# alpc91/SGRL

Measured on AMD Instinct MI355X. Metric: env-steps/sec (whole node) + SET-actor fwd us/step, 3d_walker mix @8192 envs/GPU, higher is better.
Workload: dtype f64 (dynamics) / f32 (SET actor, obs); 1 GPU; 3D_Walker++ 8 variants x 1024 envs per GPU (config 3), random U(-1,1) actions, auto-reset, SET actor forward on every step, random-init weights; envs_per_gpu=8192, obs_max_len=287, action_max_len=21, replay_gather=none (single rank)

## Files before the change

### sgrl_amd/_lib.py

```python
import ctypes
import os
import subprocess

_HERE = os.path.dirname(os.path.abspath(__file__))
LIB_PATH = os.environ.get("SGRL_HIP_LIB", os.path.join(_HERE, "libsgrl_hip.so"))
CSRC = os.path.join(_HERE, "csrc")
SOURCES = ["engine.hip", "set_actor.hip", "train_gemm.hip", "render.hip", "swat_actor.hip", "smp_actor.hip", "replay_sample.hip", "eval_record.hip", "explore_actions.hip", "scene.hip", "mlp_actor.hip", "mlp_train.hip", "mlp_optim.hip", "mlp_batch.hip", "smp_train.hip", "td3_loss.hip", "dropout.hip"]

_lib = None

_i32p = ctypes.POINTER(ctypes.c_int32)
_f64p = ctypes.POINTER(ctypes.c_double)


class SgrlError(RuntimeError):
    pass


HDR_DIM_FIELDS = (1, 2, 3, 4, 5, 6, 7, 8, 9, 16, 18)
LIGHT_NV = 12
ITAB_GLOBAL = set(x for x in os.environ.get("SGRL_BUILD_ITAB_GLOBAL", "humanoid").split(",") if x and x != "none")
PAIR_NV = {"walker": 15, "hopper": 15}


def default_max_rows(model):
    return 256


def spec_families():
    from . import mjcf, model_pack
    from .env_spec import env_spec_for
    fam = {}
    for n in mjcf.list_assets():
        m = mjcf.load_asset(n)
        ib, _ = model_pack.pack_model(m, spec=env_spec_for(n), max_rows=default_max_rows(m))
        d = tuple(int(ib[i]) for i in HDR_DIM_FIELDS)
        fam.setdefault(n.split("_")[1], set()).add(d)
    out = []
    for key in sorted(fam):
        itab = 1 if key in ITAB_GLOBAL else 0
        out.append((len(out), 2, [d + (0 if itab else (1 if d[3] <= PAIR_NV.get(key, LIGHT_NV) else 0),) for d in sorted(fam[key])], itab))
    for key in sorted(fam):
        light = sorted(d for d in fam[key] if d[3] <= LIGHT_NV)
        if light:
            out.append((len(out), 4, [d + (0,) for d in light], 0))
    return out


def hash_text(t):
    import zlib
    return zlib.crc32(t.encode())


def _write_if_changed(path, text):
    if not os.path.exists(path) or open(path).read() != text:
        with open(path, "w") as f:
            f.write(text)


def build(verbose=False):
    from concurrent.futures import ThreadPoolExecutor
    fams = spec_families()
    table = ("// generated by sgrl_amd/_lib.py build() from sgrl_amd/assets/models\n"
             "// SGRL_FAMILY(id, waves per SIMD, members, int tables in global memory)   SGRL_MEMBER(family, slot, nbody, njnt, nq, nv, nu, ngeom, npair, integrator, frame_skip, max_rows, solver, pair)\n")
    for i, w, dims, itab in fams:
        table += "SGRL_FAMILY(%d, %d, %d, %d)\n" % (i, w, len(dims), itab)
        table += "".join("SGRL_MEMBER(%d, %d, %s)\n" % (i, k, ", ".join(str(x) for x in d)) for k, d in enumerate(dims))
    _write_if_changed(os.path.join(CSRC, "spec_table.inc"), table)
    hdrs = [os.path.join(CSRC, f) for f in os.listdir(CSRC) if f.endswith((".h", ".inc"))]
    hdrs += [os.path.join(_HERE, "..", "include", f) for f in ("sgrl.h", "sgrl_model.h", "sgrl_set.h", "sgrl_swat.h", "sgrl_smp.h", "sgrl_train.h", "sgrl_render.h", "sgrl_replay.h", "sgrl_eval.h", "sgrl_explore.h", "sgrl_mlp.h")
             if os.path.exists(os.path.join(_HERE, "..", "include", f))]
    newest_hdr = max(os.path.getmtime(d) for d in hdrs)
    objdir = os.path.join(_HERE, "..", "build", "obj")
    os.makedirs(objdir, exist_ok=True)
    base = ["hipcc", "--offload-arch=gfx950", "-O3", "-std=c++17", "-fPIC", "-fno-slp-vectorize"]
    jobs = []
    for sname in SOURCES:
        src = os.path.join(CSRC, sname)
        if os.path.exists(src):
            jobs.append((os.path.join(objdir, sname.replace(".hip", ".o")), src, []))
    spec_src = os.path.join(CSRC, "step_spec.hip")
    for i, w, dims, itab in fams:
        members = ",".join("DimsFixed<%s>" % ",".join(str(x) for x in d) for d in dims)
        flags = ["-DSGRL_SPEC_ID=%d" % i, "-DSGRL_SPEC_WAVES=%d" % w, "-DSGRL_SPEC_FAMILY=" + members]
        if itab:
            flags.append("-DSGRL_ITAB_GLOBAL=1")
        tag = "%08x" % (hash_text(members + str(w) + ("g" if itab else "")) & 0xFFFFFFFF)
        jobs.append((os.path.join(objdir, "family_%d_%s.o" % (i, tag)), spec_src, flags))

    def compile_one(job):
        obj, src, flags = job
        if os.path.exists(obj) and os.path.getmtime(obj) >= max(newest_hdr, os.path.getmtime(src)):
            return False
        cmd = base + flags + ["-c", "-o", obj, src]
        if verbose:
            print(" ".join(cmd), flush=True)
        subprocess.check_call(cmd)
        return True

    with ThreadPoolExecutor(max_workers=min(8, os.cpu_count() or 1)) as pool:
        rebuilt = list(pool.map(compile_one, jobs))
    objs = [j[0] for j in jobs]
    for f in os.listdir(objdir):
        if f.endswith(".o") and os.path.join(objdir, f) not in objs:
            os.remove(os.path.join(objdir, f))
    if any(rebuilt) or not os.path.exists(LIB_PATH) or os.path.getmtime(LIB_PATH) < max(os.path.getmtime(o) for o in objs):
        cmd = ["hipcc", "--offload-arch=gfx950", "-shared", "-fPIC", "-o", LIB_PATH] + objs
        if verbose:
            print(" ".join(cmd[:8]), "... (%d objects)" % len(objs), flush=True)
        subprocess.check_call(cmd)
    return LIB_PATH


def lib():
    global _lib
    if _lib is not None:
        return _lib
    if not os.path.exists(LIB_PATH):
        raise SgrlError("HIP extension %s is missing: run `python -c 'import __graft_entry__ as g; g.build()'` "
                        "(no CPU fallback exists)" % LIB_PATH)
    import torch
    try:
        L = ctypes.CDLL(LIB_PATH)
    except OSError as e:
        raise SgrlError("cannot load %s: %s" % (LIB_PATH, e))
    L.sgrl_last_error.restype = ctypes.c_char_p
    L.sgrl_version.restype = ctypes.c_char_p
    L.sgrl_engine_create.restype = ctypes.c_int
    L.sgrl_engine_create.argtypes = [ctypes.c_int, ctypes.POINTER(_i32p), _i32p, ctypes.POINTER(_f64p), _i32p, _i32p,
                                     ctypes.c_int, ctypes.c_int, ctypes.c_uint64, ctypes.c_uint32, ctypes.c_int,
                                     ctypes.POINTER(ctypes.c_void_p)]
    L.sgrl_engine_destroy.argtypes = [ctypes.c_void_p]
    L.sgrl_engine_destroy.restype = None
    for name in ("sgrl_num_envs", "sgrl_record_stride", "sgrl_lds_bytes", "sgrl_launch_groups", "sgrl_fixed_dim_groups", "sgrl_paired_envs"):
        getattr(L, name).argtypes = [ctypes.c_void_p]
        getattr(L, name).restype = ctypes.c_int
    vp = ctypes.c_void_p
    L.sgrl_reset.argtypes = [vp, vp, vp, vp]
    L.sgrl_step.argtypes = [vp, vp, vp, vp, vp, vp, vp, vp, vp, ctypes.c_int, vp]
    L.sgrl_refresh.argtypes = [vp, vp, vp, vp]
    L.sgrl_get_records.argtypes = [vp, vp, vp]
    L.sgrl_set_records.argtypes = [vp, vp, vp]
    L.sgrl_time_steps.argtypes = [vp, vp, vp, vp, vp, ctypes.c_int, vp, ctypes.POINTER(ctypes.c_float)]
    ci = ctypes.c_int
    L.sgrl_pack_transitions.argtypes = [vp, ci, vp, ci, vp, ci, vp, vp, vp, vp, vp, vp, ci, ci, ci, vp]
    L.sgrl_ingest_rows.argtypes = [vp, ci, ci, ci, vp, vp, ci, vp]
    L.sgrl_ingest_block.argtypes = [vp, ci, ci, ci, vp, ci, vp, vp, vp, vp, vp]
    L.sgrl_round_record.argtypes = [vp, vp, vp, vp, vp, vp, vp, vp, vp, ci, ci, vp]
    L.sgrl_ingest_ws_words.argtypes = [ci]
    L.sgrl_ingest_ws_words.restype = ctypes.c_int64
    _lib = L
    return L


EXPLORE_GAUSS, EXPLORE_UNIFORM = 0, 1


def bind_explore(L):
    if getattr(L, "_explore_bound", False):
        return L
    vp, ci, cf = ctypes.c_void_p, ctypes.c_int, ctypes.c_float
    L.sgrl_explore_actions.argtypes = [vp, ci, vp, ci, vp, ci, ci, ctypes.c_int64, ctypes.c_uint64, ctypes.c_uint64, ci, cf, cf, cf, vp]
    L.sgrl_explore_actions.restype = ci
    L.sgrl_explore_actions_launches.argtypes = []
    L.sgrl_explore_actions_launches.restype = ci
    L.sgrl_explore_last_error.argtypes = []
    L.sgrl_explore_last_error.restype = ctypes.c_char_p
    L._explore_bound = True
    return L


EXPORTS = ["sgrl_engine_create", "sgrl_engine_destroy", "sgrl_num_envs", "sgrl_record_stride", "sgrl_lds_bytes", "sgrl_launch_groups", "sgrl_fixed_dim_groups", "sgrl_paired_envs",
           "sgrl_reset", "sgrl_step", "sgrl_get_records", "sgrl_set_records", "sgrl_refresh", "sgrl_time_steps", "sgrl_pack_transitions", "sgrl_round_record", "sgrl_ingest_rows", "sgrl_ingest_block", "sgrl_ingest_ws_words",
           "sgrl_last_error", "sgrl_version"]


def check(rc, what):
    if rc != 0:
        raise SgrlError("%s failed (%d): %s" % (what, rc, lib().sgrl_last_error().decode()))
```

### sgrl_amd/csrc/wave_hip.h

```cpp
#pragma once
#include <hip/hip_runtime.h>

#include "../../include/sgrl_model.h"

namespace sgrl {

template <int CTRL>
__device__ __forceinline__ double dpp_move(double x) {
  int lo = __double2loint(x), hi = __double2hiint(x);
  lo = __builtin_amdgcn_update_dpp(0, lo, CTRL, 0xF, 0xF, false);
  hi = __builtin_amdgcn_update_dpp(0, hi, CTRL, 0xF, 0xF, false);
  return __hiloint2double(hi, lo);
}
__device__ __forceinline__ double read_lane(double x, int l) {
  const int lo = __builtin_amdgcn_readlane(__double2loint(x), l);
  const int hi = __builtin_amdgcn_readlane(__double2hiint(x), l);
  return __hiloint2double(hi, lo);
}
__device__ __forceinline__ double wave_sum(double x) {
  x += dpp_move<0xB1>(x);
  x += dpp_move<0x4E>(x);
  x += dpp_move<0x141>(x);
  x += dpp_move<0x140>(x);
  return (read_lane(x, 0) + read_lane(x, 16)) + (read_lane(x, 32) + read_lane(x, 48));
}
__device__ __forceinline__ double wave_max(double x) {
  x = fmax(x, dpp_move<0xB1>(x));
  x = fmax(x, dpp_move<0x4E>(x));
  x = fmax(x, dpp_move<0x141>(x));
  x = fmax(x, dpp_move<0x140>(x));
  return fmax(fmax(read_lane(x, 0), read_lane(x, 16)), fmax(read_lane(x, 32), read_lane(x, 48)));
}

struct DimsAny {
  static constexpr bool kFixed = false;
  static constexpr bool kPair = false;
  __device__ static __forceinline__ void apply(int32_t*) {}
  template <class M> __device__ static __forceinline__ int hdr_const(const M& m, int idx) { return m.hdr[idx]; }
};
struct DimsAny;
template <int NB, int NJ, int NQ, int NV, int NU, int NG, int NP, int INTEG, int FSKIP, int MAXROWS, int SOLVER, int PAIR = 0>
struct DimsFixed {
  static constexpr bool kFixed = true;
  static constexpr int kNv = NV;
  static constexpr bool kPair = PAIR != 0;
  static_assert(PAIR == 0 || NV <= 15, "two-environments-per-wavefront instances are built for at most 15 dofs");
  __device__ static __forceinline__ void apply(int32_t* hdr) {
    hdr[SGRL_H_NBODY] = NB; hdr[SGRL_H_NJNT] = NJ; hdr[SGRL_H_NQ] = NQ; hdr[SGRL_H_NV] = NV; hdr[SGRL_H_NU] = NU;
    hdr[SGRL_H_NGEOM] = NG; hdr[SGRL_H_NPAIR] = NP; hdr[SGRL_H_INTEGRATOR] = INTEG; hdr[SGRL_H_FRAME_SKIP] = FSKIP;
    hdr[SGRL_H_MAX_ROWS] = MAXROWS; hdr[SGRL_H_SOLVER] = SOLVER;
  }
  template <class M> __device__ static __forceinline__ int hdr_const(const M& m, int idx) {
    return idx == SGRL_H_INTEGRATOR ? INTEG : (idx == SGRL_H_SOLVER ? SOLVER : (idx == SGRL_H_FRAME_SKIP ? FSKIP : m.hdr[idx]));
  }
};

typedef double sgrl_v4d __attribute__((ext_vector_type(4)));
#ifndef SGRL_AFF_MFMA_MIN
#define SGRL_AFF_MFMA_MIN 8
#endif
#ifndef SGRL_TRMM_MFMA_MIN
#define SGRL_TRMM_MFMA_MIN 9
#endif

template <int NVCAP, class D = DimsAny>
struct HipWaveT {
  static constexpr bool kFixedDims = D::kFixed;
  template <class M> __device__ static __forceinline__ int hdr_const(const M& m, int idx) { return D::hdr_const(m, idx); }
  int lane;
#ifdef SGRL_PHASE_PROF
  long long t_last = 0;
  unsigned long long* prof = nullptr;
  __device__ __forceinline__ void tick(int id) {
    const long long t = __builtin_readcyclecounter();
    if (id >= 0 && prof && lane == 0) prof[id] += (unsigned long long)(t - t_last);
    t_last = __builtin_readcyclecounter();
  }
#endif
  __device__ __forceinline__ HipWaveT() : lane(threadIdx.x & 63) {}
  __device__ __forceinline__ void fence_lane() { asm volatile("" : "+v"(lane)); }
  template <class T> __device__ __forceinline__ T fenced(T v) {
    int t = __builtin_amdgcn_readfirstlane((int)(unsigned)(__UINTPTR_TYPE__)v);
    asm volatile("" : "+s"(t));
    return (T)(__UINTPTR_TYPE__)(unsigned)t;
  }
  template <class F> __device__ __forceinline__ void lanes(int n, F f) {
    for (int i = lane; i < n; i += 64) f(i);
    __syncthreads();
  }
  template <class F> __device__ __forceinline__ void lanes_from(int lo, int hi, F f) {
    for (int i = lo + lane; i < hi; i += 64) f(i);
    __syncthreads();
  }
  template <class F> __device__ __forceinline__ double sum(int n, F f) {
    double p = 0.0;
    for (int i = lane; i < n; i += 64) p += f(i);
    return wave_sum(p);
  }
  __device__ __forceinline__ int pgs(int n_in, int nv_in, const double* Y, int ldy, const double* b, const double* R,
                                      const double* idg, double* f, double* v, int iters_in,
                                      double thresh) {
    const int n = __builtin_amdgcn_readfirstlane(n_in), nv = __builtin_amdgcn_readfirstlane(nv_in);
    const int iters = __builtin_amdgcn_readfirstlane(iters_in);
    const bool rowl = lane < n, dofl = lane < nv;
    double rb = rowl ? b[lane] : 0.0, rR = rowl ? R[lane] : 0.0;
    double ridg = rowl ? idg[lane] : 0.0, rf = rowl ? f[lane] : 0.0;
    const double rdg = rowl ? 1.0 / ridg : 0.0;
    double vv = 0.0;
    for (int r = 0; r < n; r++) {
      const double fr = read_lane(rf, r);
      if (dofl) vv += Y[r * ldy + lane] * fr;
    }
    int it = 0;
    for (; it < iters; it++) {
      double change = 0.0;
      double ynext = dofl ? Y[lane] : 0.0;
      for (int r = 0; r < n; r++) {
        const double y = ynext;
        if (r + 1 < n) ynext = dofl ? Y[(r + 1) * ldy + lane] : 0.0;
        const double dot = wave_sum(y * vv);
        const double fr = read_lane(rf, r);
        const double res = read_lane(rb, r) + read_lane(rR, r) * fr + dot;
        double fn = fr - res * read_lane(ridg, r);
        fn = fn < 0.0 ? 0.0 : fn;
        const double df = fn - fr;
        vv += y * df;
        if (lane == r) rf = fn;
        change = fmax(change, fabs(df) * read_lane(rdg, r));
      }
      if (change < thresh) { it++; break; }
    }
    if (rowl) f[lane] = rf;
    if (dofl) v[lane] = vv;
    __syncthreads();
    return it;
  }
  __device__ __forceinline__ int pgs_big(int n_in, int nv_in, const double* Y, int ldy, const double* b, const double* R,
                                          const double* idg, double* f, double* v, int iters_in, double thresh) {
    const int n = __builtin_amdgcn_readfirstlane(n_in), nv = __builtin_amdgcn_readfirstlane(nv_in);
    const int iters = __builtin_amdgcn_readfirstlane(iters_in);
    const bool dofl = lane < nv;
    const int dl = dofl ? lane : 0;
    double vv = 0.0;
    for (int r = 0; r < n; r++) {
      const double fr = f[r];
      const double y = Y[r * ldy + dl];
      if (dofl) vv += y * fr;
    }
    int it = 0;
    for (; it < iters; it++) {
      double change = 0.0;
      double yn = Y[dl], bn = b[0], Rn = R[0], in_ = idg[0], fn_ = f[0];
      for (int r = 0; r < n; r++) {
        const double y = dofl ? yn : 0.0, br = bn, Rr = Rn, ir = in_, fr = fn_;
        if (r + 1 < n) { yn = Y[(r + 1) * ldy + dl]; bn = b[r + 1]; Rn = R[r + 1]; in_ = idg[r + 1]; fn_ = f[r + 1]; }
        const double dot = wave_sum(y * vv);
        const double res = br + Rr * fr + dot;
        double fnew = fr - res * ir;
        fnew = fnew < 0.0 ? 0.0 : fnew;
        const double df = fnew - fr;
        vv += y * df;
        if (lane == 0) f[r] = fnew;
        change = fmax(change, fabs(df) / ir);
      }
      __syncthreads();
      if (change < thresh) { it++; break; }
    }
    if (dofl) v[lane] = vv;
    __syncthreads();
    return it;
  }
  template <int NMAX>
  __device__ __forceinline__ void chol_inv_reg(int n, double* P, double minval) {
    const bool act = lane < n;
    const int li = act ? lane : 0;
    double* rowp = P + li * (li + 1) / 2;
    double a[NMAX + 1];
#pragma unroll
    for (int k = 0; k < NMAX; k++) a[k + 1] = rowp[k < li ? k : li];
    double mydj = 0.0;
#pragma unroll
    for (int j = 0; j < NMAX; j++) {
      if (j < n) {
        const double c = a[j + 1];
        double pj = read_lane(c, j);
        pj = pj < minval ? minval : pj;
        const double dj = rsqrt(pj);
        const double l = c * dj;
        mydj = lane == j ? dj : mydj;
        const double lm = lane > j ? l * dj : 0.0;
        a[j] = lane == j ? 1.0 : 0.0;
#pragma unroll
        for (int c2 = 0; c2 <= j; c2++) a[c2] -= lm * read_lane(a[c2], j);
#pragma unroll
        for (int k = j + 1; k < NMAX; k++) a[k + 1] -= l * read_lane(l, k);
      }
    }
    if (act) {
#pragma unroll
      for (int k = NMAX - 1; k >= 0; k--) rowp[k < li ? k : li] = a[k] * mydj;
    }
    __syncthreads();
  }
  __device__ __forceinline__ bool chol_inv_packed(int n_in, double* P, double minval) {
    const int n = __builtin_amdgcn_readfirstlane(n_in);
    if (NVCAP >= 9 && n <= 9) chol_inv_reg<9>(n, P, minval);
    else if (NVCAP >= 12 && n <= 12) chol_inv_reg<12>(n, P, minval);
    else if (NVCAP >= 15 && n <= 15) chol_inv_reg<15>(n, P, minval);
    else if (NVCAP >= 18 && n <= 18) chol_inv_reg<18>(n, P, minval);
    else if (NVCAP >= 21 && n <= 21) chol_inv_reg<21>(n, P, minval);
    else if (NVCAP >= 24 && n <= 24) chol_inv_reg<24>(n, P, minval);
    else return false;
    return true;
  }
  template <int NMAX>
  __device__ __forceinline__ void trmm_rows_reg(int nrhs, int n, const double* T, double* Y, int ldy) {
    constexpr int NH = (NMAX + 1) / 2;
    const int h = lane & 1;
    for (int r0 = 0; r0 < nrhs; r0 += 32) {
      const int r = r0 + (lane >> 1);
      const bool act = r < nrhs;
      double* y = Y + (act ? r : nrhs - 1) * ldy;
      double jr[NH];
#pragma unroll
      for (int u = 0; u < NH; u++) {
        const int c = 2 * u + h;
        const double v = y[c < n ? c : n - 1];
        jr[u] = c < n ? v : 0.0;
      }
#pragma unroll
      for (int d = (NMAX - 1) | 1; d >= 1; d -= 2) {
        if (d - 1 < n) {
          const double* Td = T + d * (d + 1) / 2 + h;
          const double* Te = T + (d - 1) * d / 2 + h;
          double s0 = 0.0, s1 = 0.0, e0 = 0.0, e1 = 0.0;
#pragma unroll
          for (int u = 0; u < NH; u++) {
            if (2 * u + 1 <= d) {
              const double td = Td[2 * u], te = Te[2 * u];
              const double tem = (2 * u + 1 <= d - 1) ? te : (h == 0 ? te : 0.0);
              if (u & 1) { s1 += td * jr[u]; e1 += tem * jr[u]; } else { s0 += td * jr[u]; e0 += tem * jr[u]; }
            }
          }
          double sd = s0 + s1, se = e0 + e1;
          sd += dpp_move<0xB1>(sd);
          se += dpp_move<0xB1>(se);
          if (act) { if (h == 0) y[d - 1] = se; else if (d < n) y[d] = sd; }
        }
      }
    }
    __syncthreads();
  }
  __device__ __forceinline__ void trmm_rows_mfma(int nrhs, int n, const double* T, double* Y, int ldy) {
    const int lo = lane & 15, hi = lane >> 4;
    const int ksteps = (n + 3) >> 2;
    for (int r0 = 0; r0 < nrhs; r0 += 16) {
      const int r = r0 + lo;
      const bool rv = r < nrhs;
      const double* yr = Y + (rv ? r : 0) * ldy;
      double b[6];
#pragma unroll
      for (int s = 0; s < 6; s++) {
        const int c = 4 * s + hi;
        const double v = yr[c < n ? c : 0];
        b[s] = (rv && c < n) ? v : 0.0;
      }
#pragma unroll
      for (int dt = 0; dt < 2; dt++) {
        if (16 * dt < n) {
          const int d = 16 * dt + lo;
          const bool dv = d < n;
          const double* Td = T + (dv ? d * (d + 1) / 2 : 0);
          sgrl_v4d acc0 = {0, 0, 0, 0}, acc1 = {0, 0, 0, 0};
#pragma unroll
          for (int s = 0; s < 6; s++) {
            if (s < ksteps && s < 4 * dt + 4) {
              const int c = 4 * s + hi;
              const double t = Td[(dv && c <= d) ? c : 0];
              const double a = (dv && c <= d) ? t : 0.0;
              if (s & 1) acc1 = __builtin_amdgcn_mfma_f64_16x16x4f64(a, b[s], acc1, 0, 0, 0);
              else acc0 = __builtin_amdgcn_mfma_f64_16x16x4f64(a, b[s], acc0, 0, 0, 0);
            }
          }
          if (rv) {
#pragma unroll
            for (int i = 0; i < 4; i++) {
              const int dd = 16 * dt + hi + 4 * i;
              if (dd < n) Y[r * ldy + dd] = acc0[i] + acc1[i];
            }
          }
        }
      }
    }
    __syncthreads();
  }
  __device__ __forceinline__ bool aff_rows(int nf_in, int nv_in, const double* Y, int ldy, const int32_t* fl, const double* eR, double* C) {
    const int nf = __builtin_amdgcn_readfirstlane(nf_in), nv = __builtin_amdgcn_readfirstlane(nv_in);
    if (nf < SGRL_AFF_MFMA_MIN) return false;
    const int lo = lane & 15, hi = lane >> 4;
    const int nt = (nf + 15) >> 4, ksteps = (nv + 3) >> 2;
    for (int ti = 0; ti < nt; ti++) {
      const int ri = 16 * ti + lo;
      const double* yi = Y + fl[ri < nf ? ri : 0] * ldy;
      for (int tj = 0; tj <= ti; tj++) {
        const int rj = 16 * tj + lo;
        const double* yj = Y + fl[rj < nf ? rj : 0] * ldy;
        sgrl_v4d acc0 = {0, 0, 0, 0}, acc1 = {0, 0, 0, 0};
        for (int s = 0; s < ksteps; s += 2) {
          const int d0 = 4 * s + hi, d1 = d0 + 4;
          const double a0 = yi[d0 < nv ? d0 : 0], b0 = yj[d0 < nv ? d0 : 0];
          const double a1 = yi[d1 < nv ? d1 : 0], b1 = yj[d1 < nv ? d1 : 0];
          acc0 = __builtin_amdgcn_mfma_f64_16x16x4f64((d0 < nv && ri < nf) ? a0 : 0.0, (d0 < nv && rj < nf) ? b0 : 0.0, acc0, 0, 0, 0);
          if (s + 1 < ksteps)
            acc1 = __builtin_amdgcn_mfma_f64_16x16x4f64((d1 < nv && ri < nf) ? a1 : 0.0, (d1 < nv && rj < nf) ? b1 : 0.0, acc1, 0, 0, 0);
        }
#pragma unroll
        for (int i = 0; i < 4; i++) {
          const int r = 16 * ti + hi + 4 * i, c = 16 * tj + lo;
          if (r < nf && c <= r) {
            double v = acc0[i] + acc1[i];
            if (r == c) v += eR[fl[r]];
            C[r * (r + 1) / 2 + c] = v;
          }
        }
      }
    }
    __syncthreads();
    return true;
  }
  __device__ __forceinline__ bool trmm_rows(int nrhs_in, int n_in, const double* T, double* Y, int ldy) {
#ifdef SGRL_NO_TRMM
    return false;
#endif
    const int n = __builtin_amdgcn_readfirstlane(n_in), nrhs = __builtin_amdgcn_readfirstlane(nrhs_in);
    if (n >= SGRL_TRMM_MFMA_MIN && n <= 24) { trmm_rows_mfma(nrhs, n, T, Y, ldy); return true; }
    if (NVCAP >= 9 && n <= 9) trmm_rows_reg<9>(nrhs, n, T, Y, ldy);
    else if (NVCAP >= 12 && n <= 12) trmm_rows_reg<12>(nrhs, n, T, Y, ldy);
    else if (NVCAP >= 15 && n <= 15) trmm_rows_reg<15>(nrhs, n, T, Y, ldy);
    else if (NVCAP >= 18 && n <= 18) trmm_rows_reg<18>(nrhs, n, T, Y, ldy);
    else if (NVCAP >= 21 && n <= 21) trmm_rows_reg<21>(nrhs, n, T, Y, ldy);
    else if (NVCAP >= 24 && n <= 24) trmm_rows_reg<24>(nrhs, n, T, Y, ldy);
    else return false;
    return true;
  }
  __device__ __forceinline__ double trsv_lower_reg(int n, const double* P, double dv, double x) {
    const double* row = P + lane * (lane + 1) / 2;
    double lnext = (lane > 0 && lane < n) ? row[0] : 0.0;
    for (int j = 0; j < n; j++) {
      const double lj = lnext;
      if (j + 1 < n) lnext = (lane > j + 1 && lane < n) ? row[j + 1] : 0.0;
      const double xj = read_lane(x, j) * read_lane(dv, j);
      x = lane == j ? xj : (lane > j ? x - lj * xj : x);
    }
    return x;
  }
  __device__ __forceinline__ double trsv_upper_reg(int n, const double* P, double dv, double x) {
    double lnext = (n > 0 && lane < n - 1) ? P[(n - 1) * n / 2 + lane] : 0.0;
    for (int i = n - 1; i >= 0; i--) {
      const double li = lnext;
      if (i > 0) lnext = lane < i - 1 ? P[(i - 1) * i / 2 + lane] : 0.0;
      const double xi = read_lane(x, i) * read_lane(dv, i);
      x = lane == i ? xi : (lane < i ? x - li * xi : x);
    }
    return x;
  }
  __device__ __forceinline__ void trsv_lower(int n_in, const double* P, const double* dinv, double* xs) {
    const int n = __builtin_amdgcn_readfirstlane(n_in);
    const double dv = lane < n ? dinv[lane] : 0.0;
    const double x = trsv_lower_reg(n, P, dv, lane < n ? xs[lane] : 0.0);
    if (lane < n) xs[lane] = x;
    __syncthreads();
  }
  __device__ __forceinline__ void trsv_upper(int n_in, const double* P, const double* dinv, double* xs) {
    const int n = __builtin_amdgcn_readfirstlane(n_in);
    const double dv = lane < n ? dinv[lane] : 0.0;
    const double x = trsv_upper_reg(n, P, dv, lane < n ? xs[lane] : 0.0);
    if (lane < n) xs[lane] = x;
    __syncthreads();
  }
  template <int SPLIT>
  __device__ __forceinline__ void trsm_rows_split(int nrhs, int n, const double* P, const double* dinv, double* Y, int ldy) {
    constexpr int PER = 64 / SPLIT;
    const int q = lane & (SPLIT - 1);
    for (int r0 = 0; r0 < nrhs; r0 += PER) {
      const int r = r0 + lane / SPLIT;
      const bool act = r < nrhs;
      double* y = Y + (act ? r : nrhs - 1) * ldy;
      double yprev = 0.0;
      for (int i = 0; i < n; i++) {
        const double* Li = P + i * (i + 1) / 2;
        double s0 = 0.0, s1 = 0.0, s2 = 0.0, s3 = 0.0;
        int j = q;
        for (; j + 3 * SPLIT < i - 1; j += 4 * SPLIT) {
          const double a0 = Li[j], a1 = Li[j + SPLIT], a2 = Li[j + 2 * SPLIT], a3 = Li[j + 3 * SPLIT];
          const double b0 = y[j], b1 = y[j + SPLIT], b2 = y[j + 2 * SPLIT], b3 = y[j + 3 * SPLIT];
          s0 -= a0 * b0; s1 -= a1 * b1; s2 -= a2 * b2; s3 -= a3 * b3;
        }
        for (; j < i - 1; j += SPLIT) s0 -= Li[j] * y[j];
        double sum = (s0 + s1) + (s2 + s3);
        if (SPLIT >= 2) sum += dpp_move<0xB1>(sum);
        if (SPLIT >= 4) sum += dpp_move<0x4E>(sum);
        double t = y[i] + sum;
        if (i > 0) t -= Li[i - 1] * yprev;
        yprev = t * dinv[i];
        if (act && q == 0) y[i] = yprev;
      }
    }
    __syncthreads();
  }
  __device__ __forceinline__ void trsm_lower_rows(int nrhs_in, int n_in, const double* P, const double* dinv, double* Y,
                                                  int ldy) {
    const int n = __builtin_amdgcn_readfirstlane(n_in), nrhs = __builtin_amdgcn_readfirstlane(nrhs_in);
    if (nrhs <= 16) trsm_rows_split<4>(nrhs, n, P, dinv, Y, ldy);
    else if (nrhs <= 32) trsm_rows_split<2>(nrhs, n, P, dinv, Y, ldy);
    else trsm_rows_split<1>(nrhs, n, P, dinv, Y, ldy);
  }
  template <class F> __device__ __forceinline__ uint64_t ballot(int n, F f) {
    const bool p = (lane < n) ? (bool)f(lane) : false;
    return (uint64_t)__ballot(p);
  }
  template <class F> __device__ __forceinline__ double maxabs(int n, F f) {
    double p = 0.0;
    for (int i = lane; i < n; i += 64) p = fmax(p, fabs(f(i)));
    return wave_max(p);
  }
};
using HipWave = HipWaveT<24>;

template <class D>
struct HipHalfPrim {
  static constexpr bool kFixedDims = D::kFixed;
  template <class M> __device__ static __forceinline__ int hdr_const(const M& m, int idx) { return D::hdr_const(m, idx); }
  int lane;
  int half;
  __device__ __forceinline__ HipHalfPrim() : lane(threadIdx.x & 31), half((threadIdx.x >> 5) & 1) {}
#ifdef SGRL_PHASE_PROF
  __device__ __forceinline__ void tick(int) {}
#endif
  __device__ __forceinline__ void fence_lane() { asm volatile("" : "+v"(lane)); }
  template <class T> __device__ __forceinline__ T fenced(T v) {
    int t = __builtin_amdgcn_readfirstlane((int)(unsigned)(__UINTPTR_TYPE__)v);
    asm volatile("" : "+s"(t));
    return (T)(__UINTPTR_TYPE__)(unsigned)t;
  }
  __device__ static __forceinline__ void sync() { __syncthreads(); }
  __device__ static __forceinline__ double bcast16(double x, int j) {
    switch (j) {
      case 0: return dpp_move<0x150>(x);   case 1: return dpp_move<0x151>(x);   case 2: return dpp_move<0x152>(x);
      case 3: return dpp_move<0x153>(x);   case 4: return dpp_move<0x154>(x);   case 5: return dpp_move<0x155>(x);
      case 6: return dpp_move<0x156>(x);   case 7: return dpp_move<0x157>(x);   case 8: return dpp_move<0x158>(x);
      case 9: return dpp_move<0x159>(x);   case 10: return dpp_move<0x15A>(x);  case 11: return dpp_move<0x15B>(x);
      case 12: return dpp_move<0x15C>(x);  case 13: return dpp_move<0x15D>(x);  case 14: return dpp_move<0x15E>(x);
      default: return dpp_move<0x15F>(x);
    }
  }
  __device__ static __forceinline__ double xor1(double x) { return dpp_move<0xB1>(x); }
  __device__ static __forceinline__ void rows_of_half(double x, double* even, double* odd) {
    const unsigned lo = (unsigned)__double2loint(x), hi = (unsigned)__double2hiint(x);
    const auto l = __builtin_amdgcn_permlane16_swap(lo, lo, false, false);
    const auto h = __builtin_amdgcn_permlane16_swap(hi, hi, false, false);
    *even = __hiloint2double((int)h[0], (int)l[0]);
    *odd = __hiloint2double((int)h[1], (int)l[1]);
  }
  __device__ static __forceinline__ double half_sum(double x) {
    x += dpp_move<0xB1>(x);
    x += dpp_move<0x4E>(x);
    x += dpp_move<0x141>(x);
    x += dpp_move<0x140>(x);
    double e, o;
    rows_of_half(x, &e, &o);
    return e + o;
  }
  __device__ static __forceinline__ double half_max(double x) {
    x = fmax(x, dpp_move<0xB1>(x));
    x = fmax(x, dpp_move<0x4E>(x));
    x = fmax(x, dpp_move<0x141>(x));
    x = fmax(x, dpp_move<0x140>(x));
    double e, o;
    rows_of_half(x, &e, &o);
    return fmax(e, o);
  }
  __device__ __forceinline__ uint32_t half_ballot(bool p) const {
    const uint64_t b = (uint64_t)__ballot(p);
    return half ? (uint32_t)(b >> 32) : (uint32_t)b;
  }
};

}
```

Measured before the change: 2.043 million env-steps/s.

## Use all 64 lanes in packed Cholesky-inverse via split-half register form

Adds two alternative wave-level forms of the in-register packed Cholesky factor-and-invert. In the "pair" form each half-wave holds alternating columns. In the "split" form one half-wave factors L while the other builds the inverse, with the column broadcast going through LDS instead of cross-lane reads. The default path now uses the split form and keeps the lane form for n<=6 or when SGRL_CHOL_LANES is set. The aim is to use the idle upper 32 lanes and replace the per-element read_lane shuffles with vector LDS loads. The cost is extra LDS traffic and wave barriers per column, plus new numerical code paths. A debug kernel and Python binding are added so the three forms can be tested in isolation.

```diff
diff --git a/include/sgrl_debug.h b/include/sgrl_debug.h
--- /dev/null
+++ b/include/sgrl_debug.h
@@ -0,0 +1,20 @@
+#ifndef SGRL_DEBUG_H
+#define SGRL_DEBUG_H
+
+#include "sgrl.h"
+
+#ifdef __cplusplus
+extern "C" {
+#endif
+
+#define SGRL_CHOL_FORM_LANES 0
+#define SGRL_CHOL_FORM_PAIR 1
+#define SGRL_CHOL_FORM_SPLIT 2
+
+int sgrl_debug_chol_inv(int n, int form, const double* P_in, double* P_out, int count, void* stream);
+const char* sgrl_debug_last_error(void);
+
+#ifdef __cplusplus
+}
+#endif
+#endif
diff --git a/sgrl_amd/_lib.py b/sgrl_amd/_lib.py
--- a/sgrl_amd/_lib.py
+++ b/sgrl_amd/_lib.py
@@ -5,7 +5,7 @@
 _HERE = os.path.dirname(os.path.abspath(__file__))
 LIB_PATH = os.environ.get("SGRL_HIP_LIB", os.path.join(_HERE, "libsgrl_hip.so"))
 CSRC = os.path.join(_HERE, "csrc")
-SOURCES = ["engine.hip", "set_actor.hip", "train_gemm.hip", "render.hip", "swat_actor.hip", "smp_actor.hip", "replay_sample.hip", "eval_record.hip", "explore_actions.hip", "scene.hip", "mlp_actor.hip", "mlp_train.hip", "mlp_optim.hip", "mlp_batch.hip", "smp_train.hip", "td3_loss.hip", "dropout.hip"]
+SOURCES = ["engine.hip", "set_actor.hip", "train_gemm.hip", "render.hip", "swat_actor.hip", "smp_actor.hip", "replay_sample.hip", "eval_record.hip", "explore_actions.hip", "scene.hip", "mlp_actor.hip", "mlp_train.hip", "mlp_optim.hip", "mlp_batch.hip", "smp_train.hip", "td3_loss.hip", "dropout.hip", "debug_chol.hip"]
 
 _lib = None
 
@@ -68,7 +68,7 @@
         table += "".join("SGRL_MEMBER(%d, %d, %s)\n" % (i, k, ", ".join(str(x) for x in d)) for k, d in enumerate(dims))
     _write_if_changed(os.path.join(CSRC, "spec_table.inc"), table)
     hdrs = [os.path.join(CSRC, f) for f in os.listdir(CSRC) if f.endswith((".h", ".inc"))]
-    hdrs += [os.path.join(_HERE, "..", "include", f) for f in ("sgrl.h", "sgrl_model.h", "sgrl_set.h", "sgrl_swat.h", "sgrl_smp.h", "sgrl_train.h", "sgrl_render.h", "sgrl_replay.h", "sgrl_eval.h", "sgrl_explore.h", "sgrl_mlp.h")
+    hdrs += [os.path.join(_HERE, "..", "include", f) for f in ("sgrl.h", "sgrl_model.h", "sgrl_set.h", "sgrl_swat.h", "sgrl_smp.h", "sgrl_train.h", "sgrl_render.h", "sgrl_replay.h", "sgrl_eval.h", "sgrl_explore.h", "sgrl_mlp.h", "sgrl_debug.h")
              if os.path.exists(os.path.join(_HERE, "..", "include", f))]
     newest_hdr = max(os.path.getmtime(d) for d in hdrs)
     objdir = os.path.join(_HERE, "..", "build", "obj")
@@ -170,6 +170,21 @@
     return L
 
 
+CHOL_FORM_LANES, CHOL_FORM_PAIR, CHOL_FORM_SPLIT = 0, 1, 2
+
+
+def bind_debug(L):
+    if getattr(L, "_debug_bound", False):
+        return L
+    vp, ci = ctypes.c_void_p, ctypes.c_int
+    L.sgrl_debug_chol_inv.argtypes = [ci, ci, vp, vp, ci, vp]
+    L.sgrl_debug_chol_inv.restype = ci
+    L.sgrl_debug_last_error.argtypes = []
+    L.sgrl_debug_last_error.restype = ctypes.c_char_p
+    L._debug_bound = True
+    return L
+
+
 EXPORTS = ["sgrl_engine_create", "sgrl_engine_destroy", "sgrl_num_envs", "sgrl_record_stride", "sgrl_lds_bytes", "sgrl_launch_groups", "sgrl_fixed_dim_groups", "sgrl_paired_envs",
            "sgrl_reset", "sgrl_step", "sgrl_get_records", "sgrl_set_records", "sgrl_refresh", "sgrl_time_steps", "sgrl_pack_transitions", "sgrl_round_record", "sgrl_ingest_rows", "sgrl_ingest_block", "sgrl_ingest_ws_words",
            "sgrl_last_error", "sgrl_version"]
diff --git a/sgrl_amd/csrc/debug_chol.hip b/sgrl_amd/csrc/debug_chol.hip
--- /dev/null
+++ b/sgrl_amd/csrc/debug_chol.hip
@@ -0,0 +1,58 @@
+#include <hip/hip_runtime.h>
+
+#include <string>
+
+#include "../../include/sgrl.h"
+#include "../../include/sgrl_debug.h"
+#include "wave_hip.h"
+
+namespace {
+
+thread_local std::string g_debug_err;
+
+int fail(int code, const std::string& msg) {
+  g_debug_err = msg;
+  return code;
+}
+
+constexpr int kNMax = 24, kTriMax = kNMax * (kNMax + 1) / 2;
+constexpr double kMinVal = 1e-15;
+
+template <int FORM>
+__global__ __launch_bounds__(64) __attribute__((amdgpu_waves_per_eu(2, 2))) void k_debug_chol_inv(int n, const double* __restrict__ P_in, double* __restrict__ P_out) {
+  __shared__ __attribute__((aligned(16))) double S[kTriMax + 2];
+  sgrl::HipWaveT<kNMax> w;
+  const int tri = n * (n + 1) / 2;
+  double* P = S + 1;
+  const double* src = P_in + (size_t)blockIdx.x * tri;
+  double* dst = P_out + (size_t)blockIdx.x * tri;
+  for (int i = w.lane; i < tri; i += 64) P[i] = src[i];
+  __syncthreads();
+  w.template chol_inv_form<FORM>(n, P, kMinVal);
+  for (int i = w.lane; i < tri; i += 64) dst[i] = P[i];
+}
+
+}
+
+extern "C" {
+
+int sgrl_debug_chol_inv(int n, int form, const double* P_in, double* P_out, int count, void* stream) {
+  if (n < 1 || n > kNMax) return fail(SGRL_ERR_ARG, "sgrl_debug_chol_inv: n must be in 1..24");
+  if (form != SGRL_CHOL_FORM_LANES && form != SGRL_CHOL_FORM_PAIR && form != SGRL_CHOL_FORM_SPLIT) return fail(SGRL_ERR_ARG, "sgrl_debug_chol_inv: unknown form");
+  if (count < 0) return fail(SGRL_ERR_ARG, "sgrl_debug_chol_inv: count < 0");
+  if (count == 0) return SGRL_OK;
+  if (!P_in || !P_out) return fail(SGRL_ERR_ARG, "sgrl_debug_chol_inv: null matrix pointer");
+  if (form == SGRL_CHOL_FORM_LANES)
+    hipLaunchKernelGGL(k_debug_chol_inv<0>, dim3((unsigned)count), dim3(64), 0, (hipStream_t)stream, n, P_in, P_out);
+  else if (form == SGRL_CHOL_FORM_SPLIT)
+    hipLaunchKernelGGL(k_debug_chol_inv<2>, dim3((unsigned)count), dim3(64), 0, (hipStream_t)stream, n, P_in, P_out);
+  else
+    hipLaunchKernelGGL(k_debug_chol_inv<1>, dim3((unsigned)count), dim3(64), 0, (hipStream_t)stream, n, P_in, P_out);
+  const hipError_t e = hipGetLastError();
+  if (e != hipSuccess) return fail(SGRL_ERR_HIP, std::string("sgrl_debug_chol_inv: ") + hipGetErrorString(e));
+  return SGRL_OK;
+}
+
+const char* sgrl_debug_last_error(void) { return g_debug_err.c_str(); }
+
+}
diff --git a/sgrl_amd/csrc/wave_hip.h b/sgrl_amd/csrc/wave_hip.h
--- a/sgrl_amd/csrc/wave_hip.h
+++ b/sgrl_amd/csrc/wave_hip.h
@@ -56,6 +56,7 @@
 };
 
 typedef double sgrl_v4d __attribute__((ext_vector_type(4)));
+typedef double sgrl_v2d __attribute__((ext_vector_type(2)));
 #ifndef SGRL_AFF_MFMA_MIN
 #define SGRL_AFF_MFMA_MIN 8
 #endif
@@ -171,7 +172,7 @@
     return it;
   }
   template <int NMAX>
-  __device__ __forceinline__ void chol_inv_reg(int n, double* P, double minval) {
+  __device__ __forceinline__ void chol_inv_reg_lanes(int n, double* P, double minval) {
     const bool act = lane < n;
     const int li = act ? lane : 0;
     double* rowp = P + li * (li + 1) / 2;
@@ -202,16 +203,148 @@
     }
     __syncthreads();
   }
-  __device__ __forceinline__ bool chol_inv_packed(int n_in, double* P, double minval) {
+  template <int NMAX>
+  __device__ __forceinline__ void chol_inv_reg_pair(int n, double* P, double minval) {
+    constexpr int NH = (NMAX + 1) / 2, NQ = (NH + 1) / 2;
+    const int h = lane >> 5, row = lane & 31;
+    const bool act = row < n;
+    const int li = act ? row : 0;
+    double* rowp = P + li * (li + 1) / 2;
+    double b[NH + 1];
+    b[0] = 0.0;
+#pragma unroll
+    for (int u = 0; u < NH; u++) {
+      const int k = 2 * u + h;
+      b[u + 1] = rowp[k < li ? k : li];
+    }
+    const int lh = ((n + 1) / 2 + 1) & ~1;
+    double* X = P + (((unsigned)(__UINTPTR_TYPE__)P >> 3) & 1u);
+    double* Xw = X + h * lh;
+    const sgrl_v2d* Xr = (const sgrl_v2d*)__builtin_assume_aligned(Xw, 16);
+    double* Xown = X + (li & 1) * lh + (li >> 1);
+    double mydj = 0.0;
+#pragma unroll
+    for (int j = 0; j < NMAX; j++) {
+      if (j < n) {
+        const int jh = j & 1, ju = j >> 1;
+        const double c = b[ju + 1];
+        double pj = read_lane(c, j + 32 * jh);
+        pj = pj < minval ? minval : pj;
+        const double dj = rsqrt(pj);
+        mydj = row == j ? dj : mydj;
+        if (h == jh) b[ju] = row == j ? 1.0 : 0.0;
+        if (h == jh && row > j && act) *Xown = c * dj;
+        if (row == j) {
+#pragma unroll
+          for (int u = 0; u < ju; u++) Xw[u] = b[u];
+          if (jh == 1 || h == 0) Xw[ju] = b[ju];
+        }
+        __builtin_amdgcn_fence(__ATOMIC_RELEASE, "wavefront");
+        __builtin_amdgcn_wave_barrier();
+        __builtin_amdgcn_fence(__ATOMIC_ACQUIRE, "wavefront");
+        const double l = *Xown;
+        const double lm = row > j ? l * dj : 0.0;
+        sgrl_v2d x[NQ];
+#pragma unroll
+        for (int q = 0; q < NQ; q++) x[q] = Xr[q];
+#pragma unroll
+        for (int u = 0; u < NH; u++) {
+          const double xu = x[u >> 1][u & 1];
+          asm volatile("" : "+v"(b[u + 1]));
+          if (u < ju || (u == ju && jh == 1)) b[u] -= lm * xu;
+          else if (u > ju) b[u + 1] -= l * xu;
+          else {
+            b[u] -= lm * xu;
+            b[u + 1] -= l * xu;
+          }
+        }
+      }
+    }
+    if (act) {
+#pragma unroll
+      for (int u = NH - 1; u >= 0; u--) {
+        const int k = 2 * u + h;
+        if (k <= li) rowp[k] = b[u] * mydj;
+      }
+    }
+    __syncthreads();
+  }
+  template <int NMAX>
+  __device__ __forceinline__ void chol_inv_reg_split(int n, double* P, double minval) {
+    constexpr int NQ = (NMAX + 1) / 2;
+    const int h = lane >> 5, idx = lane & 31;
+    const bool act = idx < n;
+    const int li = act ? idx : 0;
+    double reg[NMAX];
+    {
+      const double* rowp = P + li * (li + 1) / 2;
+#pragma unroll
+      for (int k = 0; k < NMAX; k++) {
+        const double v = rowp[k < li ? k : li];
+        reg[k] = h == 0 ? v : 0.0;
+      }
+    }
+    const int lh = (n + 1) & ~1;
+    double* X = P + (((unsigned)(__UINTPTR_TYPE__)P >> 3) & 1u);
+    double* Xown = X + li;
+    const sgrl_v2d* Xr = (const sgrl_v2d*)__builtin_assume_aligned(X + h * lh, 16);
+#pragma unroll
+    for (int j = 0; j < NMAX; j++) {
+      if (j < n) {
+        const double c = reg[j];
+        double pj = read_lane(c, j);
+        pj = pj < minval ? minval : pj;
+        const double dj = rsqrt(pj);
+        const double l = c * dj;
+        if (h == 0 && idx > j && act) { Xown[0] = l; Xown[lh] = l * dj; }
+        const double t = idx == j ? 1.0 : c;
+        const double A = h == 0 ? l : t;
+        reg[j] = (t - 0.0 * t) * dj;
+        __builtin_amdgcn_fence(__ATOMIC_RELEASE, "wavefront");
+        __builtin_amdgcn_wave_barrier();
+        __builtin_amdgcn_fence(__ATOMIC_ACQUIRE, "wavefront");
+        sgrl_v2d x[NQ];
+#pragma unroll
+        for (int q = (j + 1) >> 1; q < NQ; q++) x[q] = Xr[q];
+#pragma unroll
+        for (int k = j + 1; k < NMAX; k++) {
+          reg[k] -= A * x[k >> 1][k & 1];
+          asm volatile("" : "+v"(reg[k]));
+        }
+      }
+    }
+    if (h == 1 && act) {
+#pragma unroll
+      for (int k = 0; k < NMAX; k++)
+        if (k < n && idx <= k) P[k * (k + 1) / 2 + idx] = reg[k];
+    }
+    __syncthreads();
+  }
+#ifndef SGRL_CHOL_LANES
+#define SGRL_CHOL_LANES 0
+#endif
+  template <int FORM, int NMAX>
+  __device__ __forceinline__ void chol_inv_reg(int n, double* P, double minval) {
+    if (FORM == 0) chol_inv_reg_lanes<NMAX>(n, P, minval);
+    else if (FORM == 1) chol_inv_reg_pair<NMAX>(n, P, minval);
+    else chol_inv_reg_split<NMAX>(n, P, minval);
+  }
+  template <int FORM>
+  __device__ __forceinline__ bool chol_inv_form(int n_in, double* P, double minval) {
     const int n = __builtin_amdgcn_readfirstlane(n_in);
-    if (NVCAP >= 9 && n <= 9) chol_inv_reg<9>(n, P, minval);
-    else if (NVCAP >= 12 && n <= 12) chol_inv_reg<12>(n, P, minval);
-    else if (NVCAP >= 15 && n <= 15) chol_inv_reg<15>(n, P, minval);
-    else if (NVCAP >= 18 && n <= 18) chol_inv_reg<18>(n, P, minval);
-    else if (NVCAP >= 21 && n <= 21) chol_inv_reg<21>(n, P, minval);
-    else if (NVCAP >= 24 && n <= 24) chol_inv_reg<24>(n, P, minval);
+    if (FORM == 1 && n <= 3) chol_inv_reg_lanes<3>(n, P, minval);
+    else if (FORM == 2 && n <= 6) chol_inv_reg_lanes<6>(n, P, minval);
+    else if (NVCAP >= 9 && n <= 9) chol_inv_reg<FORM, 9>(n, P, minval);
+    else if (NVCAP >= 12 && n <= 12) chol_inv_reg<FORM, 12>(n, P, minval);
+    else if (NVCAP >= 15 && n <= 15) chol_inv_reg<FORM, 15>(n, P, minval);
+    else if (NVCAP >= 18 && n <= 18) chol_inv_reg<FORM, 18>(n, P, minval);
+    else if (NVCAP >= 21 && n <= 21) chol_inv_reg<FORM, 21>(n, P, minval);
+    else if (NVCAP >= 24 && n <= 24) chol_inv_reg<FORM, 24>(n, P, minval);
     else return false;
     return true;
+  }
+  __device__ __forceinline__ bool chol_inv_packed(int n_in, double* P, double minval) {
+    return chol_inv_form<SGRL_CHOL_LANES ? 0 : 2>(n_in, P, minval);
   }
   template <int NMAX>
   __device__ __forceinline__ void trmm_rows_reg(int nrhs, int n, const double* T, double* Y, int ldy) {
diff --git a/sgrl_amd/debug.py b/sgrl_amd/debug.py
--- /dev/null
+++ b/sgrl_amd/debug.py
@@ -0,0 +1,20 @@
+import ctypes
+
+import torch
+
+from . import _lib
+
+CHOL_FORM_LANES, CHOL_FORM_PAIR, CHOL_FORM_SPLIT = _lib.CHOL_FORM_LANES, _lib.CHOL_FORM_PAIR, _lib.CHOL_FORM_SPLIT
+
+
+def chol_inv(P, n, form):
+    tri = n * (n + 1) // 2
+    if P.dtype != torch.float64 or not P.is_cuda or P.dim() != 2 or P.shape[1] != tri or not P.is_contiguous():
+        raise _lib.SgrlError("chol_inv: P must be a contiguous float64 [count, %d] tensor on the GPU" % tri)
+    L = _lib.bind_debug(_lib.lib())
+    out = torch.empty_like(P)
+    rc = L.sgrl_debug_chol_inv(int(n), int(form), ctypes.c_void_p(P.data_ptr()), ctypes.c_void_p(out.data_ptr()), int(P.shape[0]),
+                               ctypes.c_void_p(torch.cuda.current_stream(P.device).cuda_stream))
+    if rc != 0:
+        raise _lib.SgrlError("sgrl_debug_chol_inv failed (%d): %s" % (rc, L.sgrl_debug_last_error().decode()))
+    return out
```

Result: no change. 2.060 million env-steps/s (median of 6 runs) (+0.8%).
